# Illumina/strelka

Measured on AMD Instinct MI355X. Metric: candidate-alignment scoring cells/s (read bases x candidate alignments; Strelka2 has no pair-HMM, SURVEY.md section 0) + germline loci/s + 40x WGS-like germline wall-clock (e2e) + 110x/40x somatic wall-clock (e2e_somatic), higher is better.
Workload: dtype f64; 1 GPU; germline chr20-style synthetic (BASELINE.json configs[1]).  Headline: scoreCandidateAlignment as one function -- per GPU per step 65536 reads of 150 bp x 87.9 candidate alignments each (5-7 candidate indels around them), from the candidate alignments the device search left (PCal) to one double each: one kernel (F5: the walk of each alignment's path + the terms of its bases, penalties and clips).  ; read_len=150

## Files before the change

### strelka_amd/csrc/read_enumerate.hip

```cpp

#include "sk_common.h"

#include "align_entry.h"
#include "read_enumerate.h"

#include <algorithm>
#include <chrono>
#include <climits>
#include <cstdio>
#include <cstdlib>
#include <cstring>
#include <vector>

using namespace skcore;

int sk_score_alignments_launch_hostleg(const sk_align_batch* b, double* dev_out_lnp, void* hip_stream);

namespace
{

static_assert(sizeof(PFrame) % 4 == 0 && sizeof(PCal) % 4 == 0, "frames move through LDS as 32-bit words");


struct EnumArgs
// ... 457 lines not shown
    if (nc == 0) return;
    int32_t wb = a.win_begin[r], we = a.win_end[r];
    if (wb > we) wb = we = 0;
    a.win_begin[r] = wb;
    int32_t len = we - wb;
    a.win_len[r] = len;
    int16_t* idx = a.ins_idx + size_t(r) * INS_CAP;
    int32_t* off = a.ins_off + size_t(r) * INS_CAP;
    int n = 0;
    for (int t = a.ins_lo[r]; t <= a.ins_hi[r]; ++t) {
        const uint32_t il = a.job.tab[t].ins_len;
        if (il == 0) continue;
        if (n >= INS_CAP) {
            a.status[r] = ST_OVERFLOW;
            n = 0;
            break;
        }
        idx[n] = int16_t(t);
        off[n] = len;
        len += int32_t(il);
        ++n;
    }
    a.n_ins[r] = n;
    a.hap_len[r] = max(len, 1);
}

__device__ int matching_indel(const PJob& j, const PCal& c, const int32_t ref_head_pos, const unsigned del_len, const unsigned ins_len,
                              const int ends_first, const int ends_second, const int path_index)
{
    if (path_index < ends_first) return c.lead;
    if (path_index > ends_second) return c.trail;
    int found = -1;
    for (int k = 0; k < c.n_indels; ++k) {
        const PIndel& ci = j.tab[c.indels[k]];
        if (ci.pos == ref_head_pos && (ci.type == SK_INDEL_INDEL || ci.type == SK_INDEL_MISMATCH) && ci.del == del_len &&
            ci.ins_len == ins_len) {
            if (found >= 0) return -2;
            found = c.indels[k];
        } else if (ci.pos > ref_head_pos) {
            break;
        }
    }
    return found >= 0 ? found : -2;
}

struct NoOpSink
{
    __device__ __forceinline__ void operator()(uint8_t, uint32_t, int32_t, bool) const {}
};

template <bool WRITE, typename SINK = NoOpSink>
__device__ int flatten_cal(const FlatArgs& a, const int r, const PCal& c, const int32_t read_len, sk_score_op* ops, SINK&& sink = SINK())
{
    const int aps = c.n_seg;
    const int32_t win_begin = a.win_begin[r];
    const int n_ins = a.n_ins[r];
    const int16_t* ins_idx = a.ins_idx + size_t(r) * INS_CAP;
    const int32_t* ins_off = a.ins_off + size_t(r) * INS_CAP;
    unsigned read_offset = 0;
    int32_t ref_head_pos = c.pos;
    int ends_first = aps, ends_second = aps;
    {
        bool is_first_match = false;
        for (int i = 0; i < aps; ++i)
            if (seg_align_match(c.path[i].type)) {
                if (!is_first_match) ends_first = i;
                is_first_match = true;
                ends_second = i;
            }
    }
    int n = 0;
    auto emit = [&](const uint8_t kind, const uint32_t len, const int32_t src, const bool penalty) {
        if (kind == SK_OP_NOBASE && !penalty) return;
        sink(kind, len, src, penalty);
        if (WRITE) {
            sk_score_op op;
            op.length = uint16_t(len);
            op.kind = kind;
            op.flags = uint8_t(penalty ? SK_OPFLAG_NONCANDIDATE_PENALTY : 0);
            op.src = src;
            ops[n] = op;
        }
        ++n;
    };
    auto insert_src = [&](const int idx, const int32_t head, const uint32_t len) -> int32_t {
        const PIndel& k = a.job.tab[idx];
        if (head < 0 || uint32_t(head) + len > k.ins_len) return -1;
        for (int i = 0; i < n_ins; ++i)
            if (ins_idx[i] == idx) return ins_off[i] + head;
        return -1;
    };
    auto is_cand = [&](const int idx) -> bool { return job_cand(a.job, idx); };

    int path_index = 0;
    while (path_index < aps) {
        bool is_swap_start = false;
        {
            bool is_insert = false, is_delete = false;
            for (int i = path_index; i < aps; ++i) {
                if (c.path[i].type == SK_SEG_INSERT) is_insert = true;
                else if (c.path[i].type == SK_SEG_DELETE) is_delete = true;
                else break;
            }
            is_swap_start = is_insert && is_delete;
        }
        unsigned n_seg = 1;
        const PSeg ps = c.path[path_index];
        if (is_swap_start || ps.type == SK_SEG_SEQ_MISMATCH) {
            unsigned del_len, ins_len;
            if (ps.type == SK_SEG_SEQ_MISMATCH) {
                del_len = ins_len = ps.length;
            } else {
                int k = path_index;
                del_len = ins_len = 0;
                for (; k < aps && (c.path[k].type == SK_SEG_INSERT || c.path[k].type == SK_SEG_DELETE); ++k) {
                    if (c.path[k].type == SK_SEG_INSERT) ins_len += c.path[k].length;
                    else del_len += c.path[k].length;
                }
                n_seg = unsigned(k - path_index);
            }
            const int key = matching_indel(a.job, c, ref_head_pos, del_len, ins_len, ends_first, ends_second, path_index);
            if (key < 0) return -1;
            int32_t head = 0;
            if (path_index < ends_first) head = int32_t(a.job.tab[key].ins_len) - int32_t(ps.length);
            const bool pen = !is_cand(key);
            if (ins_len > 0) {
                if (ins_len > 0xffffu) return -1;
                const int32_t src = insert_src(key, head, ins_len);
                if (src < 0) return -1;
                emit(SK_OP_BASES, ins_len, src, pen);
            } else {
                emit(SK_OP_NOBASE, 0, 0, pen);
            }
        } else if (seg_align_match(ps.type)) {
            emit(SK_OP_BASES, ps.length, ref_head_pos - win_begin, false);
        } else if (ps.type == SK_SEG_INSERT) {
            const int key = matching_indel(a.job, c, ref_head_pos, 0, ps.length, ends_first, ends_second, path_index);
            if (key < 0) return -1;
            int32_t head = 0;
            if (path_index < ends_first) head = int32_t(a.job.tab[key].ins_len) - int32_t(ps.length);
            const int32_t src = insert_src(key, head, ps.length);
            if (src < 0) return -1;
            emit(SK_OP_BASES, ps.length, src, !is_cand(key));
        } else if (ps.type == SK_SEG_DELETE) {
            const int key = matching_indel(a.job, c, ref_head_pos, ps.length, 0, ends_first, ends_second, path_index);
            if (key < 0) return -1;
            emit(SK_OP_NOBASE, 0, 0, !is_cand(key));
        } else if (ps.type == SK_SEG_SKIP || ps.type == SK_SEG_HARD_CLIP) {
        } else if (ps.type == SK_SEG_SOFT_CLIP) {
            emit(SK_OP_SOFT_CLIP, ps.length, 0, false);
        } else {
            return -1;
        }
        for (unsigned i = 0; i < n_seg; ++i) {
            const PSeg s = c.path[path_index];
            if (seg_align_match(s.type)) {
                read_offset += s.length;
                ref_head_pos += int32_t(s.length);
            } else if (s.type == SK_SEG_DELETE || s.type == SK_SEG_SKIP) {
                ref_head_pos += int32_t(s.length);
            } else if (s.type == SK_SEG_INSERT || s.type == SK_SEG_SOFT_CLIP) {
                read_offset += s.length;
            }
            path_index++;
        }
    }
    if (int64_t(read_offset) != int64_t(read_len)) return -1;
    return n;
}

__global__ __launch_bounds__(64) void op_count_kernel(const FlatArgs a)
{
    const int c = blockIdx.x * blockDim.x + threadIdx.x;
    if (c >= a.n_cals) return;
    const int r = read_of_cal(a, c);
    const PCal& cal = a.pool[a.list[c]];
    const int n = flatten_cal<false>(a, r, cal, int32_t(a.read_off[r + 1] - a.read_off[r]), nullptr);
    if (n < 0) a.status[r] = ST_FAIL;
    a.n_ops[c] = n < 0 ? 0 : n;
}

__global__ __launch_bounds__(64) void pool_fill_kernel(const FlatArgs a)
{
    const int r = blockIdx.x;
    if (a.cal_off[r + 1] == a.cal_off[r]) return;
    uint8_t* hap = a.hap_code + a.hap_off[r];
    const int32_t P = int32_t(a.hap_off[r + 1] - a.hap_off[r]);
    const int32_t wb = a.win_begin[r];
    const int n_ins = a.n_ins[r];
    const int16_t* idx = a.ins_idx + size_t(r) * INS_CAP;
    const int32_t* off = a.ins_off + size_t(r) * INS_CAP;
    const int32_t win_len = a.win_len[r];
    for (int32_t i = threadIdx.x; i < P; i += 64) {
        uint8_t v = SK_BAM_ANY;
        if (i < win_len) {
            const int32_t p = wb + i;
            const bool outside = (p < a.ref_offset || p >= a.ref_offset + a.ref_len);
            if (outside && a.ref_outside) atomicAdd(a.ref_outside, 1);
            v = outside ? uint8_t(SK_BAM_ANY) : code_of(a.ref[p - a.ref_offset]);
        }
        for (int k = 0; k < n_ins; ++k) {
            const PIndel& d = a.job.tab[idx[k]];
            if (i >= off[k] && i < off[k] + int32_t(d.ins_len)) v = code_of(a.ins_pool[d.ins_off + uint32_t(i - off[k])]);
        }
        hap[i] = v;
    }
}

__global__ __launch_bounds__(64) void flatten_kernel(const FlatArgs a)
{
    constexpr int REC_DW = int(sizeof(PCal) / 4), REC_STRIDE = REC_DW | 1;
    static_assert(sizeof(PCal) % 4 == 0 && REC_DW <= 128, "a record is at most two dwords per lane");
    __shared__ uint32_t s_cal[64 * REC_STRIDE];
    const int lane = threadIdx.x;
    const int c0 = blockIdx.x * blockDim.x;
    const int c = c0 + lane;
    const int nc = min(64, a.n_cals - c0);
    const int src_k = (lane < nc) ? a.list[c0 + lane] : 0;
    for (int k = 0; k < nc; ++k) {
        const uint32_t* __restrict__ src = reinterpret_cast<const uint32_t*>(a.pool + __shfl(src_k, k));
        uint32_t* __restrict__ dst = reinterpret_cast<uint32_t*>(a.cals + (c0 + k));
        for (int j = lane; j < REC_DW; j += 64) {
            const uint32_t v = src[j];
            s_cal[k * REC_STRIDE + j] = v;
            dst[j] = v;
        }
    }
    __syncthreads();
    if (c >= a.n_cals) return;
    const int r = read_of_cal(a, c);
    const PCal& cal = *reinterpret_cast<const PCal*>(s_cal + lane * REC_STRIDE);
    if (a.status[r] != ST_OK) return;
    (void)flatten_cal<true>(a, r, cal, int32_t(a.read_off[r + 1] - a.read_off[r]), a.ops + a.op_off[c]);
    for (int i = 0; i < cal.n_indels; ++i) (void)job_cand(a.job, cal.indels[i]);
    if (cal.lead >= 0) (void)job_cand(a.job, cal.lead);
    if (cal.trail >= 0) (void)job_cand(a.job, cal.trail);
}

constexpr int F5_MAX_READ = 256;
constexpr int ONE_WAIT_MAX_READS = 16384;
constexpr int F5_MAX_POOL = 768;
#ifndef F5_SORT
#define F5_SORT 1
#endif
constexpr int F5_TAB = 32;

static_assert(F5_TAB <= 64, "the table copy is a lane an entry");

struct FusedScoreArgs
{
    FlatArgs f;
    const uint8_t* read_qual;
    const SkTables* tab;
    double* scores;
    unsigned* err;
    int32_t* n_unhandled;
    int32_t write_cals;
    unsigned long long* dbg;
    unsigned* queue;
};

constexpr int F5_SEGS = 16, F5_INDELS = 8;
constexpr int F5_SLOT = (F5_SEGS + 1) | 1;
__device__ __forceinline__ int f5_ent_word(const int k) { return k; }
constexpr int F5_ROW = 3;

struct F5Tab
{
    int32_t pos;
    uint32_t del, ins_len;
    uint32_t type_cand;
    int32_t ins_at;
};

template <int MAXR>
struct F5Lds
{
    uint8_t read[MAXR + 12];
    uint8_t hap[F5_MAX_POOL + 12];
    double row[(MAXR + 8) * F5_ROW];
    uint32_t slot[64 * F5_SLOT];
    F5Tab tab[F5_TAB];
};
static_assert(sizeof(F5Lds<152>) <= 10240, "sixteen waves of the short-read form to a CU");
static_assert(3 * 4 * sizeof(F5Lds<F5_MAX_READ>) <= 160 * 1024, "three four-wave blocks of the long-read form to a CU");
static_assert((152 + 12) % 4 == 0 && (F5_MAX_READ + 12) % 4 == 0 && (F5_MAX_POOL + 12) % 4 == 0, "the byte arrays' words stay aligned");
static_assert(INS_CAP <= 64, "a lane an insert");

struct F5Rec
{
    uint32_t w0, w1, w2;
    uint64_t types;
    uint64_t l0, l1, l2, l3;
    uint64_t ind;
    int ind_lo;
    __device__ __forceinline__ int32_t pos() const { return int32_t(w0); }
    __device__ __forceinline__ int lead() const { return int(int16_t(w1 & 0xffffu)); }
    __device__ __forceinline__ int trail() const { return int(int16_t(w1 >> 16)); }
    __device__ __forceinline__ int n_seg() const { return int((w2 >> 8) & 0xffu); }
    __device__ __forceinline__ int n_indels() const { return int((w2 >> 16) & 0xffu); }
    __device__ __forceinline__ int indel(const int k) const { return ind_lo + int(unsigned(ind >> (6 * k)) & 63u); }
};
static_assert(F5_TAB <= 64 && 6 * F5_INDELS <= 64, "an indel index in 6 bits, eight in one value");

template <typename LDS>
__device__ __forceinline__ int f5_walk_selects(LDS& S, const F5Rec c, const bool has, const int tab_lo, const int32_t win_begin, uint8_t* consulted,
                                               const int32_t L, const int32_t P, uint32_t* const myslot)
{
    constexpr uint64_t N1 = 0x1111111111111111ull;
    const uint64_t types = c.types, p_l0 = c.l0, p_l1 = c.l1, p_l2 = c.l2, p_l3 = c.l3;
    const int aps = has ? c.n_seg() : 0;
    auto eq4 = [=](const unsigned v) -> uint64_t {
        uint64_t x = types ^ (N1 * v);
        x |= x >> 1;
        x |= x >> 2;
        return ~x & N1;
    };
    auto seg_len = [=](const int i) -> unsigned {
        const uint64_t lo = (i & 4) ? p_l1 : p_l0, hi = (i & 4) ? p_l3 : p_l2;
        return unsigned(((i & 8) ? hi : lo) >> (16 * (i & 3))) & 0xffffu;
    };
    const uint64_t in_path = (aps >= 16) ? N1 : (((1ull << (4 * aps)) - 1ull) & N1);
    const uint64_t M4 = (eq4(SK_SEG_MATCH) | eq4(SK_SEG_SEQ_MATCH) | eq4(SK_SEG_SEQ_MISMATCH)) & in_path;
    const uint64_t I4 = eq4(SK_SEG_INSERT) & in_path, D4 = eq4(SK_SEG_DELETE) & in_path;
    const int ends_first = M4 ? (__builtin_ctzll(M4) >> 2) : aps, ends_second = M4 ? ((63 - __builtin_clzll(M4)) >> 2) : aps;
    const int ni = c.n_indels();
    int ni_wave = 0;
#pragma unroll
    for (int k = 1; k <= F5_INDELS; ++k) ni_wave = __any(ni >= k) ? k : ni_wave;
    int32_t k_pos[F5_INDELS];
    uint32_t k_pack[F5_INDELS];
    bool bad = false;
#pragma unroll
    for (int k = 0; k < F5_INDELS; ++k) {
        k_pos[k] = INT_MIN;
        k_pack[k] = 0xffffffffu;
        if (k < ni_wave) {
            const F5Tab& ci = S.tab[((k < ni) ? c.indel(k) : tab_lo) - tab_lo];
            const unsigned ty = ci.type_cand & 0xffu;
            const bool kind = (ty == SK_INDEL_INDEL || ty == SK_INDEL_MISMATCH);
            if (k < ni) {
                k_pos[k] = ci.pos;
                if (kind) {
                    k_pack[k] = (ci.del << 16) | ci.ins_len;
                    bad = bad || ci.del >= 0xffffu || ci.ins_len >= 0xffffu;
                }
            }
        }
    }
    int pi = 0, n_ent = 0;
    int32_t pos = 0, ref_head_pos = c.pos();
    unsigned npen = 0;
    for (;;) {
        const bool live = pi < aps && !bad;
        if (!__any(live)) break;
        const int sh = 4 * (pi & 15);
        const unsigned ty = unsigned(types >> sh) & 15u, ln = seg_len(pi & 15);
        const uint64_t not_run = ~((I4 | D4) >> sh) & N1;
        const int run4 = not_run ? __builtin_ctzll(not_run) : 64;
        const uint64_t run_set = (run4 >= 64) ? ~0ull : ((1ull << run4) - 1ull);
        const bool is_swap = live && ((I4 >> sh) & run_set) != 0ull && ((D4 >> sh) & run_set) != 0ull;
        const bool is_match = (ty == SK_SEG_MATCH || ty == SK_SEG_SEQ_MATCH), is_clip = (ty == SK_SEG_SOFT_CLIP);
        const bool is_indel_seg = is_swap || ty == SK_SEG_SEQ_MISMATCH || ty == SK_SEG_INSERT || ty == SK_SEG_DELETE;
        unsigned del_len = (ty == SK_SEG_INSERT) ? 0u : ln, ins_len = (ty == SK_SEG_DELETE) ? 0u : ln;
        int n_seg = 1;
        unsigned read_step = (is_match || ty == SK_SEG_SEQ_MISMATCH || ty == SK_SEG_INSERT || is_clip) ? ln : 0u;
        unsigned ref_step = (is_match || ty == SK_SEG_SEQ_MISMATCH || ty == SK_SEG_DELETE || ty == SK_SEG_SKIP) ? ln : 0u;
        if (is_swap) {
            n_seg = run4 >> 2;
            del_len = ins_len = 0;
            for (int k = 0; k < n_seg; ++k) {
                const unsigned l = seg_len((pi + k) & 15);
                if ((I4 >> (4 * ((pi + k) & 15))) & 1ull) ins_len += l;
                else del_len += l;
            }
            read_step = ins_len;
            ref_step = del_len;
        }
        const unsigned asked = (del_len << 16) | ins_len;
        const bool askable = del_len < 0xffffu && ins_len < 0xffffu;
        int k_found = 0, n_found = 0;
        bool open = true;
#pragma unroll
        for (int k = 0; k < F5_INDELS; ++k) {
            if (k < ni_wave) {
                const bool m = open && k_pos[k] == ref_head_pos && k_pack[k] == asked;
                k_found = m ? k : k_found;
                n_found += m ? 1 : 0;
                open = open && (m || k_pos[k] <= ref_head_pos);
            }
        }
        int key = (n_found == 1) ? c.indel(k_found) : -2;
        key = (pi < ends_first) ? c.lead() : (pi > ends_second) ? c.trail() : key;
        const bool key_ok = key >= 0;
        const F5Tab te = S.tab[(key_ok ? key : tab_lo) - tab_lo];
        const bool indel_ok = live && is_indel_seg && key_ok;
        if (indel_ok && consulted) consulted[key] = 1;
        const bool pen = is_indel_seg && (te.type_cand >> 8) == 0u;
        const int32_t head = (pi < ends_first) ? int32_t(te.ins_len) - int32_t(ln) : 0;
        const bool ins_bases = is_indel_seg && ins_len > 0u;
        const bool ins_ok = ins_len <= 0xffffu && head >= 0 && uint32_t(head) + ins_len <= te.ins_len && te.ins_at >= 0;
        const bool bases = ins_bases || is_match;
        const int32_t src = ins_bases ? te.ins_at + head : ref_head_pos - win_begin;
        const unsigned len = ins_bases ? ins_len : ln;
        const bool known = is_indel_seg || is_match || is_clip || ty == SK_SEG_SKIP || ty == SK_SEG_HARD_CLIP;
        bool fail = !known || (is_indel_seg && (!key_ok || !askable)) || (ins_bases && !ins_ok);
        const bool entry = (bases || (is_clip && !is_indel_seg)) && len > 0u;
        if (entry) {
            fail = fail || pos + int32_t(len) > L || (bases && (src < 0 || int64_t(src) + int64_t(len) > int64_t(P)));
            const int hidx = bases ? int(src) - pos : 0;
            fail = fail || n_ent > F5_SEGS || npen > 4u || hidx < -256 || hidx > 3839;
            if (live && !fail) myslot[f5_ent_word(n_ent)] = unsigned(pos) | (npen << 9) | (bases ? 0u : 1u << 15) | (unsigned(hidx + 256) << 16);
        }
        if (live) {
            bad = fail;
            n_ent += entry ? 1 : 0;
            npen = entry ? (pen ? 1u : 0u) : npen + (pen ? 1u : 0u);
            pos += int32_t(read_step);
            ref_head_pos += int32_t(ref_step);
            pi += n_seg;
        }
    }
    if (!has) return 0;
    if (bad || pos != L || n_ent > F5_SEGS || npen > 4u) return -1;
    myslot[f5_ent_word(n_ent)] = unsigned(L) | (npen << 9) | (256u << 16);
    return n_ent + 1;
}

template <typename LDS>
__device__ __forceinline__ double f5_sum(LDS& S, const uint32_t* const myslot, const int n_ent, const double ln_noncand, const double ln_quarter)
{
    double lnp = 0.0;
    const unsigned char* rows = reinterpret_cast<const unsigned char*>(S.row);
    int e = 0, p = 0, stop = 0, hidx = 0;
    uint32_t cur = myslot[f5_ent_word(0)], nxt = myslot[f5_ent_word(1)];
    auto next_op = [&]() -> bool {
        const bool adv = (p >= stop);
        const int start = int(cur & 0x1ffu), next_start = int(nxt & 0x1ffu);
        const unsigned np = adv ? ((cur >> 9) & 63u) : 0u;
        const bool clip = adv && (cur & (1u << 15)) != 0u;
        if (__builtin_amdgcn_ballot_w64(np != 0u || clip) != 0ull) {
            const double l1 = __dadd_rn(lnp, ln_noncand);
            lnp = (np >= 1u) ? l1 : lnp;
            const double l2 = __dadd_rn(lnp, ln_noncand);
            lnp = (np >= 2u) ? l2 : lnp;
            const double l3 = __dadd_rn(lnp, ln_noncand);
            lnp = (np >= 3u) ? l3 : lnp;
            const double l4 = __dadd_rn(lnp, ln_noncand);
            lnp = (np >= 4u) ? l4 : lnp;
            const double lc = __dadd_rn(lnp, __dmul_rn(double(unsigned(next_start - start)), ln_quarter));
            lnp = clip ? lc : lnp;
        }
        if (adv && e + 1 >= n_ent) return true;
        p = adv ? (clip ? next_start : start) : p;
        stop = adv ? next_start : stop;
        hidx = adv ? int(cur >> 16) - 256 : hidx;
        e = adv ? e + 1 : e;
        cur = adv ? nxt : cur;
        nxt = myslot[f5_ent_word(e + 1)];
        return false;
    };
    if (next_op()) return lnp;
    for (;;) {
        {
            const int m = stop - p;
            const int mm = (m > 8) ? 8 : m;
            const int ph = p + hidx;
            const uint32_t* const rw = reinterpret_cast<const uint32_t*>(S.read + (p & ~3));
            const uint32_t* const hw = reinterpret_cast<const uint32_t*>(S.hap + (ph & ~3));
            const uint32_t r0 = rw[0], r1 = rw[1], r2 = rw[2], h0 = hw[0], h1 = hw[1], h2 = hw[2];
            const uint32_t R[2] = {__builtin_amdgcn_alignbyte(r1, r0, unsigned(p)), __builtin_amdgcn_alignbyte(r2, r1, unsigned(p))};
            const uint32_t H[2] = {__builtin_amdgcn_alignbyte(h1, h0, unsigned(ph)), __builtin_amdgcn_alignbyte(h2, h1, unsigned(ph))};
            const uint64_t past = (mm >= 8) ? 0ull : (0x1818181818181818ull << (8 * mm));
            constexpr uint32_t B0F = 0x0f0f0f0fu, B10 = 0x10101010u;
            uint32_t sel[2];
#pragma unroll
            for (int h = 0; h < 2; ++h) {
                const uint32_t x = (R[h] ^ H[h]) + B0F;
                uint32_t pm = uint32_t(past >> (32 * h));
                __asm__("" : "+v"(pm));
                sel[h] = (B10 & ~pm & x) | (~B10 & pm);
                __asm__("" : "+v"(sel[h]));
            }
            const unsigned base = __umul24(unsigned(8 * F5_ROW), unsigned(p));
            double v[8];
#pragma unroll
            for (int u = 0; u < 8; ++u) {
                const unsigned at = base + unsigned(8 * F5_ROW * u) + ((sel[u >> 2] >> (8 * (u & 3))) & 0xffu);
                v[u] = *reinterpret_cast<const double*>(rows + at);
            }
#pragma unroll
            for (int u = 0; u < 8; ++u) lnp = __dadd_rn(lnp, v[u]);
            p += mm;
        }
        if (next_op()) break;
    }
    return lnp;
}

__device__ __forceinline__ void f5_wave_sync()
{
    __builtin_amdgcn_fence(__ATOMIC_RELEASE, "workgroup");
    __builtin_amdgcn_wave_barrier();
    __builtin_amdgcn_fence(__ATOMIC_ACQUIRE, "workgroup");
}

template <int MAXR, bool TIMING>
__device__ __forceinline__ void f5_read(const FusedScoreArgs& fa, const int r, F5Lds<MAXR>& S)
{
    auto now = [&]() -> unsigned long long { return TIMING ? (unsigned long long)clock64() : 0ull; };
    const FlatArgs& a = fa.f;
    const int lane = threadIdx.x & 63;
    const int c0 = a.cal_off[r], c1 = a.cal_off[r + 1];
    const int ncr = c1 - c0;
    if (ncr == 0 || a.status[r] != ST_OK) return;
    unsigned long long stamp[8];
    stamp[0] = now();
    const unsigned long long wall0 = TIMING ? (unsigned long long)wall_clock64() : 0ull;
    for (int i = 1; i < 8; ++i) stamp[i] = 0;
    const int64_t ro = a.read_off[r];
    const int32_t L = int32_t(a.read_off[r + 1] - ro);
    const int32_t P = a.hap_len[r];
    if (L > MAXR || P > F5_MAX_POOL) {
        if (lane == 0) atomicAdd(fa.n_unhandled, 1);
        return;
    }
    const int32_t win_begin = a.win_begin[r];
    const int n_ins = a.n_ins[r];
    int my_ins_idx = -1;
    int32_t my_ins_off = 0;
    {
        const int16_t* idx = a.ins_idx + size_t(r) * INS_CAP;
        const int32_t* off = a.ins_off + size_t(r) * INS_CAP;
        int32_t my_ins_len = 0;
        uint32_t my_ins_src = 0;
        if (lane < n_ins) {
            const int t_idx = idx[lane];
            my_ins_idx = t_idx;
            my_ins_off = off[lane];
            my_ins_len = int32_t(a.job.tab[t_idx].ins_len);
            my_ins_src = a.job.tab[t_idx].ins_off;
        }
        const int32_t win_len = a.win_len[r];
        for (int32_t i = lane; i < P + 8; i += 64) {
            uint8_t v = SK_BAM_ANY;
            if (i < win_len) {
                const int32_t p = win_begin + i;
                const bool outside = (p < a.ref_offset || p >= a.ref_offset + a.ref_len);
                if (outside && a.ref_outside) atomicAdd(a.ref_outside, 1);
                v = outside ? uint8_t(SK_BAM_ANY) : code_of(a.ref[p - a.ref_offset]);
            }
            S.hap[i] = v;
        }
        f5_wave_sync();
        for (int k = 0; k < n_ins; ++k) {
            const int32_t o = __builtin_amdgcn_readlane(my_ins_off, k), n = __builtin_amdgcn_readlane(my_ins_len, k);
            const uint32_t src = uint32_t(__builtin_amdgcn_readlane(int(my_ins_src), k));
            for (int32_t i = lane; i < n; i += 64)
                if (o + i < P) S.hap[o + i] = code_of(a.ins_pool[src + uint32_t(i)]);
        }
        const SkTables* __restrict__ T = fa.tab;
        for (int32_t i = lane; i < L + 12; i += 64) {
            unsigned q = 0;
            uint8_t code = SK_BAM_ANY;
            if (i < L) {
                code = a.read_code[ro + i];
                q = fa.read_qual[ro + i];
                if (q > 70u) {
                    atomicOr(fa.err, unsigned(SK_DEVERR_QSCORE));
                    q = 70u;
                }
            }
            S.read[i] = code & 15u;
            if (i < L + 8) {
                const unsigned c = code & 15u;
                const bool adds = i < L && c != 15u;
                const double agree = adds ? T->q2lncompe[q] : 0.0;
                S.row[F5_ROW * i] = agree;
                S.row[F5_ROW * i + 1] = 0.0;
                S.row[F5_ROW * i + 2] = !adds ? 0.0 : (c == 0u) ? agree : T->q2mis[q];
            }
        }
    }
    const double ln_quarter = fa.tab->ln_quarter, ln_noncand = fa.tab->ln_noncand;

    uint8_t* const order = S.hap + ((P + 8 + 3) & ~3);
    const bool sorted_order = (F5_SORT != 0) && ncr > 64 && ncr <= 256 && ((P + 8 + 3) & ~3) + ncr <= int(sizeof(S.hap));
    if (sorted_order) {
        int seg_of[4];
#pragma unroll
        for (int k = 0; k < 4; ++k) {
            const int j = lane + 64 * k;
            seg_of[k] = (j < ncr) ? int(a.n_seg8[c0 + j]) : -1;
            seg_of[k] = min(seg_of[k], F5_SEGS + 1);
        }
        unsigned present = 0;
#pragma unroll
        for (int k = 0; k < 4; ++k) present |= (seg_of[k] >= 0) ? (1u << seg_of[k]) : 0u;
#pragma unroll
        for (int d = 32; d >= 1; d >>= 1) present |= unsigned(__shfl_xor(int(present), d));
        present = unsigned(__builtin_amdgcn_readfirstlane(int(present)));
        int at = 0;
        while (present != 0u) {
            const int v = 31 - __builtin_clz(present);
            present &= ~(1u << v);
#pragma unroll
            for (int k = 0; k < 4; ++k) {
                const uint64_t m = __ballot(seg_of[k] == v);
                if (seg_of[k] == v) order[at + __popcll(m & ((1ull << lane) - 1ull))] = uint8_t(lane + 64 * k);
                at += __popcll(m);
            }
        }
    }

    for (int j0 = 0; j0 < ncr; j0 += 64) {
        const int nc = min(64, ncr - j0);
        f5_wave_sync();
        const unsigned long long ta = now();
        if (j0 == 0) stamp[1] = ta;
        const bool has = lane < nc;
        uint32_t* const myslot = S.slot + lane * F5_SLOT;
        bool fits = true;
        const int my_j = has ? (sorted_order ? int(order[j0 + lane]) : j0 + lane) : 0;
        F5Rec rec;
        rec.w0 = rec.w1 = rec.w2 = 0;
        rec.types = 0;
        rec.l0 = rec.l1 = rec.l2 = rec.l3 = 0;
        rec.ind = 0;
        rec.ind_lo = 0;
        uint64_t ind_raw0 = 0, ind_raw1 = 0;
        if (has) {
            const PCal* src = a.pool + a.list[c0 + my_j];
            const uint4* s4 = reinterpret_cast<const uint4*>(src);
            const uint4 q0 = s4[0], q1 = s4[1], q2 = s4[2], q3 = s4[3], q4 = s4[4];
            const uint32_t* si = reinterpret_cast<const uint32_t*>(src->indels);
            const uint32_t i0 = si[0], i1 = si[1], i2 = si[2], i3 = si[3];
            ind_raw0 = uint64_t(i0) | (uint64_t(i1) << 32);
            ind_raw1 = uint64_t(i2) | (uint64_t(i3) << 32);
            rec.w0 = q0.x;
            rec.w1 = q0.y;
            rec.w2 = q0.z;
            const unsigned nseg = (q0.z >> 8) & 0xffu, nind = (q0.z >> 16) & 0xffu;
            fits = (nseg <= unsigned(F5_SEGS) && nind <= unsigned(F5_INDELS));
            uint64_t types = 0;
            bool odd_type = false;
            auto pack4 = [&](const uint32_t a0, const uint32_t a1, const uint32_t a2, const uint32_t a3, const int first) -> uint64_t {
                types |= (uint64_t(a0 & 15u) | (uint64_t(a1 & 15u) << 4) | (uint64_t(a2 & 15u) << 8) | (uint64_t(a3 & 15u) << 12)) << (4 * first);
                odd_type = odd_type || (unsigned(first) < nseg && (a0 & 0xffffu) > 15u) || (unsigned(first + 1) < nseg && (a1 & 0xffffu) > 15u) ||
                           (unsigned(first + 2) < nseg && (a2 & 0xffffu) > 15u) || (unsigned(first + 3) < nseg && (a3 & 0xffffu) > 15u);
                return uint64_t(a0 >> 16) | (uint64_t(a1 >> 16) << 16) | (uint64_t(a2 >> 16) << 32) | (uint64_t(a3 >> 16) << 48);
            };
            rec.l0 = pack4(q0.w, q1.x, q1.y, q1.z, 0);
            rec.l1 = pack4(q1.w, q2.x, q2.y, q2.z, 4);
            rec.l2 = pack4(q2.w, q3.x, q3.y, q3.z, 8);
            rec.l3 = pack4(q3.w, q4.x, q4.y, q4.z, 12);
            rec.types = types;
            fits = fits && !odd_type;
        }
        auto raw_indel = [&](const int k) -> int { return int(int16_t(((k & 4) ? ind_raw1 : ind_raw0) >> (16 * (k & 3)))); };
        int tab_lo = 0;
        {
            int lo = INT_MAX, hi = INT_MIN;
            if (has && fits) {
                auto add = [&](const int i) {
                    lo = min(lo, i);
                    hi = max(hi, i);
                };
                const int ni = rec.n_indels();
                for (int i = 0; i < ni; ++i) add(raw_indel(i));
                if (rec.lead() >= 0) add(rec.lead());
                if (rec.trail() >= 0) add(rec.trail());
            }
#pragma unroll
            for (int d = 32; d > 0; d >>= 1) {
                lo = min(lo, __shfl_xor(lo, d));
                hi = max(hi, __shfl_xor(hi, d));
            }
            const int n_tab = (lo <= hi) ? hi - lo + 1 : 0;
            if (__any(has && !fits) || (n_tab > 0 && lo < 0) || n_tab > F5_TAB) {
                if (lane == 0) atomicAdd(fa.n_unhandled, 1);
                return;
            }
            tab_lo = n_tab ? lo : 0;
            uint64_t ind = 0;
#pragma unroll
            for (int k = 0; k < F5_INDELS; ++k) ind |= uint64_t(unsigned(raw_indel(k) - tab_lo) & 63u) << (6 * k);
            rec.ind = ind;
            rec.ind_lo = tab_lo;
            if (lane < n_tab) {
                const PIndel& g = a.job.tab[tab_lo + lane];
                F5Tab e;
                e.pos = g.pos;
                e.del = g.del;
                e.ins_len = g.ins_len;
                e.type_cand = unsigned(g.type) | (unsigned(g.cand) << 8);
                e.ins_at = -1;
                S.tab[lane] = e;
            }
            f5_wave_sync();
            if (my_ins_idx >= tab_lo && my_ins_idx < tab_lo + n_tab) S.tab[my_ins_idx - tab_lo].ins_at = my_ins_off;
        }
        f5_wave_sync();
        const unsigned long long tc = now();
        stamp[2] += tc - ta;
        int n_ent = 0;
        bool bad = false;
        {
            const unsigned long long tA0 = now();
            n_ent = f5_walk_selects(S, rec, has, tab_lo, win_begin, a.job.consulted, L, P, myslot);
            const unsigned long long tA1 = now();
            stamp[7] += tA1 - tA0;
            bad = n_ent < 0;
            if (has) {
                if (a.job.consulted) {
                    const int ni = rec.n_indels();
                    for (int i = 0; i < ni; ++i) a.job.consulted[rec.indel(i)] = 1;
                    if (rec.lead() >= 0) a.job.consulted[rec.lead()] = 1;
                    if (rec.trail() >= 0) a.job.consulted[rec.trail()] = 1;
                }
                if (bad) a.status[r] = ST_FAIL;
            }
            (void)tA1;
        }
        __builtin_amdgcn_wave_barrier();
        const unsigned long long td = now();
        stamp[4] += td - tc;
        if (has && !bad) {
            const double lnp = f5_sum(S, myslot, n_ent, ln_noncand, ln_quarter);
            fa.scores[c0 + my_j] = lnp;
        }
        stamp[5] += now() - td;
    }
    if (fa.dbg && lane == 0) {
        stamp[6] = now();
        stamp[3] = TIMING ? (unsigned long long)wall_clock64() - wall0 : 0ull;
        for (int i = 0; i < 8; ++i) fa.dbg[size_t(r) * 8 + i] = stamp[i];
    }
}

template <int MAXR, bool TIMING, int WAVES>
__global__ __launch_bounds__(64 * WAVES) __attribute__((amdgpu_waves_per_eu(4, 4))) void flatten_score_kernel(const FusedScoreArgs fa, const int n_reads)
{
    __shared__ __attribute__((aligned(16))) F5Lds<MAXR> S[WAVES];
    const int wave = threadIdx.x >> 6, lane = threadIdx.x & 63;
    for (;;) {
        int r = 0;
        if (lane == 0) r = int(atomicAdd(&fa.queue[0], 1u));
        r = __builtin_amdgcn_readfirstlane(r);
        if (r >= n_reads) break;
        f5_read<MAXR, TIMING>(fa, r, S[wave]);
        f5_wave_sync();
    }
    if (lane == 0) {
        __threadfence();
        if (atomicAdd(&fa.queue[1], 1u) == gridDim.x * unsigned(WAVES) - 1u) {
            fa.queue[0] = 0u;
            fa.queue[1] = 0u;
        }
    }
}

template <int MAXR, bool TIMING>
static void launch_flatten_score_t(const int n_reads, hipStream_t st, const FusedScoreArgs& fs)
{
    static const int waves = [] { const char* e = std::getenv("SK_F5_WAVES"); return e ? std::atoi(e) : 0; }();
    constexpr int DEFAULT_WAVES = (sizeof(F5Lds<MAXR>) * 16 <= 160 * 1024) ? 8 : 4;
    const int w = waves > 0 ? waves : DEFAULT_WAVES;
    static const int grid_env = [] { const char* e = std::getenv("SK_F5_GRID"); return e ? std::atoi(e) : 0; }();
    constexpr int WAVES_PER_CU = int((160 * 1024) / sizeof(F5Lds<MAXR>)) >= 16 ? 16 : int((160 * 1024) / sizeof(F5Lds<MAXR>));
    auto grid = [&](const int wpb) {
        const int resident = grid_env > 0 ? grid_env : 256 * std::max(1, WAVES_PER_CU / wpb);
        return dim3(unsigned(std::max(1, std::min(resident, (n_reads + wpb - 1) / wpb))));
    };
    if (w == 16 && MAXR <= 152) SK_LAUNCH((flatten_score_kernel<152, TIMING, 16>), grid(16), dim3(1024), 0, st, fs, n_reads);
    else if (w >= 8) SK_LAUNCH((flatten_score_kernel<MAXR, TIMING, 8>), grid(8), dim3(512), 0, st, fs, n_reads);
    else if (w == 4) SK_LAUNCH((flatten_score_kernel<MAXR, TIMING, 4>), grid(4), dim3(256), 0, st, fs, n_reads);
    else if (w == 2) SK_LAUNCH((flatten_score_kernel<MAXR, TIMING, 2>), grid(2), dim3(128), 0, st, fs, n_reads);
    else SK_LAUNCH((flatten_score_kernel<MAXR, TIMING, 1>), grid(1), dim3(64), 0, st, fs, n_reads);
}

static void launch_flatten_score(const int n_reads, hipStream_t st, const FusedScoreArgs& fs)
{
    const bool short_reads = fs.f.max_read_len <= 152, timing = fs.dbg != nullptr;
    if (short_reads && !timing) launch_flatten_score_t<152, false>(n_reads, st, fs);
    else if (short_reads) launch_flatten_score_t<152, true>(n_reads, st, fs);
    else if (!timing) launch_flatten_score_t<F5_MAX_READ, false>(n_reads, st, fs);
    else launch_flatten_score_t<F5_MAX_READ, true>(n_reads, st, fs);
}

__global__ __launch_bounds__(64) void gather_cals_kernel(const PCal* __restrict__ pool, const int32_t* __restrict__ list, const int32_t n_cals,
                                                         PCal* __restrict__ cals)
{
    constexpr int REC_DW = int(sizeof(PCal) / 4);
    const int lane = threadIdx.x;
    const int c0 = blockIdx.x * 64;
    const int nc = min(64, n_cals - c0);
    const int src_k = (lane < nc) ? list[c0 + lane] : 0;
    for (int k0 = 0; k0 < nc; k0 += 16) {
        uint32_t v0[16], v1[16];
#pragma unroll
        for (int u = 0; u < 16; ++u) {
            const int k = k0 + u;
            const uint32_t* __restrict__ src = reinterpret_cast<const uint32_t*>(pool + __shfl(src_k, (k < nc) ? k : 0));
            v0[u] = (k < nc) ? src[lane] : 0u;
            v1[u] = (k < nc && lane + 64 < REC_DW) ? src[lane + 64] : 0u;
        }
#pragma unroll
        for (int u = 0; u < 16; ++u) {
            const int k = k0 + u;
            if (k < nc) {
                uint32_t* __restrict__ dst = reinterpret_cast<uint32_t*>(cals + (c0 + k));
                dst[lane] = v0[u];
                if (lane + 64 < REC_DW) dst[lane + 64] = v1[u];
            }
        }
    }
}


__device__ inline bool f3_emit_entries(const FlatArgs& a, const int c, const int r, const uint8_t* hap, const int32_t L, const int32_t P,
                                       uint32_t* ent, int& n_ent)
{
    const int W = a.evmask_words;
    uint32_t* mask = a.evmask + int64_t(r) * W;
    const bool read_ok = (L >= 0 && L <= SK_ENT_MAX_READ_LEN && L <= a.max_read_len && P >= 0 && P <= SK_ENT_MAX_POOL);
    auto col_at = [&](const int idx) -> unsigned { return (idx >= 0 && idx < P) ? sk_ent_col_index(hap[idx]) : unsigned(SK_ENT_ZERO_COL); };
    const int64_t k0 = a.op_off[c], k1 = a.op_off[c + 1];
    const int nslots = int(k1 - k0) + 2;
    for (int i = 0; i < nslots; ++i) ent[i] = SK_ENT_END;
    bool complex_cal = !read_ok;
    int e = 0, pos = 0;
    unsigned npen = 0;
    auto emit = [&](const unsigned np, const bool clip, const int hidx) {
        if (np > 7u || hidx + SK_ENT_HIDX_BIAS < 0 || hidx + SK_ENT_HIDX_BIAS > 2047) complex_cal = true;
        if (complex_cal) return;
        ent[e++] = unsigned(pos) | (np << 10) | (clip ? 1u << 13 : 0u) | (col_at(hidx + pos) << 15) | (col_at(hidx + pos + 1) << 18) |
                   (unsigned(hidx + SK_ENT_HIDX_BIAS) << 21);
        if (pos > 0 && pos <= L) atomicOr(&mask[pos >> 5], 1u << (pos & 31));
    };
    for (int64_t kk = k0; kk < k1 && !complex_cal; ++kk) {
        const sk_score_op op = a.ops[kk];
        const int len = int(op.length);
        const unsigned pen = op.flags & SK_OPFLAG_NONCANDIDATE_PENALTY;
        if ((op.kind == SK_OP_BASES || op.kind == SK_OP_SOFT_CLIP) && len > 0) {
            if (pos >= int(SK_ENT_END)) {
                complex_cal = true;
                break;
            }
            const bool bases = (op.kind == SK_OP_BASES);
            if (bases && (op.src < 0 || int64_t(op.src) + len > P)) complex_cal = true;
            emit(npen, !bases, bases ? int(op.src) - pos : P - pos);
            pos += len;
            npen = pen;
        } else {
            npen += pen;
        }
    }
    if (!complex_cal) {
        if (pos != L || pos >= int(SK_ENT_END)) complex_cal = true;
        else emit(npen, false, P - pos);
    }
    if (complex_cal) {
        for (int i = 0; i < nslots; ++i) ent[i] = SK_ENT_END;
        ent[0] = SK_ENT_COMPLEX;
        atomicOr(&a.addmask[int64_t(r) * W + (W - 1)], 1u << 31);
        n_ent = 0;
        return true;
    }
    uint32_t* am = a.addmask + int64_t(r) * W;
    for (int i = 0; i < e; ++i)
        if (ent[i] & SK_ENT_ADD_BITS) {
            const unsigned p = ent[i] & SK_ENT_POS_MASK;
            atomicOr(&am[p >> 5], 1u << (p & 31));
        }
    n_ent = e;
    return false;
}

__device__ inline void f3_columns_serial(const FlatArgs& a, const int c, const int r, const uint8_t* hap, const int32_t L, const int32_t P,
                                         const uint32_t* ent, const int e)
{
    const int W = a.evmask_words;
    auto col_at = [&](const int idx) -> unsigned { return (idx >= 0 && idx < P) ? sk_ent_col_index(hap[idx]) : unsigned(SK_ENT_ZERO_COL); };
    const int64_t k0 = a.op_off[c], k1 = a.op_off[c + 1];
    const int ncr = a.cal_off[r + 1] - a.cal_off[r], j = c - a.cal_off[r];
    uint32_t* cm = reinterpret_cast<uint32_t*>(a.colmat) + a.colmat_off[r] + j;
    const uint8_t* read = a.read_code + a.read_off[r];
    constexpr uint32_t NONE_WORD = 0x11111111u * SK_SEL_NONE;
    uint32_t word = NONE_WORD;
    int wk = 0;
    int pos = 0;
    const int nch = (L + 7) >> 3;
    int ei = 0;
    bool needs_entries = false;
    auto flag_at = [&](const int i) -> unsigned {
        while (ei < e && int(ent[ei] & SK_ENT_POS_MASK) < i) ++ei;
        if (ei < e && int(ent[ei] & SK_ENT_POS_MASK) == i && (ent[ei] & SK_ENT_ADD_BITS)) {
            const bool simple = ((ent[ei] >> 10) & 7u) == 1u && !(ent[ei] & (1u << 13)) && i < 8 * nch;
            if (simple) return 4u;
            needs_entries = true;
        }
        return 0u;
    };
    auto put = [&](const int i, const unsigned sel) {
        const int k8 = i >> 3;
        if (k8 != wk) {
            cm[int64_t(wk) * ncr] = word;
            for (int q = wk + 1; q < k8; ++q) cm[int64_t(q) * ncr] = NONE_WORD;
            word = NONE_WORD;
            wk = k8;
        }
        const unsigned shift = 8u * (unsigned(i) & 3u) + ((i & 4) ? 4u : 0u);
        word = (word & ~(0xfu << shift)) | (sel << shift);
    };
    for (int64_t kk = k0; kk < k1; ++kk) {
        const sk_score_op op = a.ops[kk];
        const int len = int(op.length);
        if (!((op.kind == SK_OP_BASES || op.kind == SK_OP_SOFT_CLIP) && len > 0)) continue;
        if (op.kind == SK_OP_BASES) {
            for (int t = 0; t < len && pos + t < L; ++t)
                put(pos + t, sk_col_selector(col_at(int(op.src) + t), read[pos + t]) | flag_at(pos + t));
        } else if (flag_at(pos)) {
        }
        pos += len;
    }
    {
        const unsigned f = flag_at(L);
        if (f) put(L, SK_SEL_NONE | f);
    }
    for (; ei < e; ++ei)
        if ((ent[ei] & SK_ENT_ADD_BITS) && int(ent[ei] & SK_ENT_POS_MASK) > L) needs_entries = true;
    if (needs_entries) atomicOr(&a.addmask[int64_t(r) * W + (W - 1)], 1u << 30);
    if (wk < nch) cm[int64_t(wk) * ncr] = word;
    for (int q = wk + 1; q < nch; ++q) cm[int64_t(q) * ncr] = NONE_WORD;
}

__global__ __launch_bounds__(64) void entries_kernel(const FlatArgs a)
{
    const int c = blockIdx.x * blockDim.x + threadIdx.x;
    if (c >= a.n_cals) return;
    const int r = read_of_cal(a, c);
    const int32_t L = int32_t(a.read_off[r + 1] - a.read_off[r]);
    const int32_t P = int32_t(a.hap_off[r + 1] - a.hap_off[r]);
    const uint8_t* hap = a.hap_code + a.hap_off[r];
    uint32_t* ent = a.entries + a.op_off[c] + 2 * int64_t(c);
    int e = 0;
    if (f3_emit_entries(a, c, r, hap, L, P, ent, e)) return;
    f3_columns_serial(a, c, r, hap, L, P, ent, e);
}

constexpr int F3W_MAX_D = 64;
constexpr int F3W_MAX_NCH = 32;
constexpr int F3W_MAX_POOL = 1024;

struct F3wLds
{
    uint8_t hap[F3W_MAX_POOL];
    uint8_t read[8 * F3W_MAX_NCH];
    uint8_t slot_of[2048];
    uint32_t delta_bits[64];
    int32_t n_slots;
    int16_t delta_of[F3W_MAX_D];
    uint32_t M[F3W_MAX_D][F3W_MAX_NCH];
    uint32_t tile[F3W_MAX_NCH][64];
};

__device__ __forceinline__ uint32_t f3w_below(const int x)
{
    const uint32_t lo = (x >= 4) ? 0x0f0f0f0fu : (uint32_t((1ull << (8 * x)) - 1ull) & 0x0f0f0f0fu);
    const uint32_t hi = (x <= 4) ? 0u : (x >= 8 ? 0xf0f0f0f0u : (uint32_t((1ull << (8 * (x - 4))) - 1ull) & 0xf0f0f0f0u));
    return lo | hi;
}

__global__ __launch_bounds__(64) void entries_wave_kernel(const FlatArgs a)
{
    __shared__ F3wLds S;
    const int r = blockIdx.x;
    const int lane = threadIdx.x;
    const int c0 = a.cal_off[r], c1 = a.cal_off[r + 1];
    const int ncr = c1 - c0;
    if (ncr == 0) return;
    const int32_t L = int32_t(a.read_off[r + 1] - a.read_off[r]);
    const int32_t P = int32_t(a.hap_off[r + 1] - a.hap_off[r]);
    const uint8_t* ghap = a.hap_code + a.hap_off[r];
    const uint8_t* gread = a.read_code + a.read_off[r];
    const int nch = (L + 7) >> 3;
    const bool fits = (L >= 0 && nch <= F3W_MAX_NCH && P >= 0 && P <= F3W_MAX_POOL);
    if (fits) {
        for (int i = lane; i < P; i += 64) S.hap[i] = ghap[i];
        for (int i = lane; i < 8 * nch; i += 64) S.read[i] = (i < L) ? gread[i] : uint8_t(15);
    }
    S.delta_bits[lane] = 0;
    if (lane == 0) S.n_slots = 0;
    __syncthreads();
    const uint8_t* hap = fits ? S.hap : ghap;

    for (int c = c0 + lane; c < c1; c += 64) {
        uint32_t* ent = a.entries + a.op_off[c] + 2 * int64_t(c);
        int e = 0;
        const bool complex_cal = f3_emit_entries(a, c, r, hap, L, P, ent, e);
        if (complex_cal) continue;
        if (!fits) {
            f3_columns_serial(a, c, r, hap, L, P, ent, e);
            continue;
        }
        int pos = 0;
        for (int64_t kk = a.op_off[c]; kk < a.op_off[c + 1]; ++kk) {
            const sk_score_op op = a.ops[kk];
            const int len = int(op.length);
            if (!((op.kind == SK_OP_BASES || op.kind == SK_OP_SOFT_CLIP) && len > 0)) continue;
            if (op.kind == SK_OP_BASES) {
                const int d = int(op.src) - pos + SK_ENT_HIDX_BIAS;
                atomicOr(&S.delta_bits[d >> 5], 1u << (d & 31));
            }
            pos += len;
        }
    }
    if (!fits) return;
    __syncthreads();
    {
        const uint32_t w = S.delta_bits[lane];
        int n = __popc(w), before = n;
#pragma unroll
        for (int d = 1; d < 64; d <<= 1) {
// ... 1269 lines not shown
```

Baseline: 757.1 billion cells/s.

## Add swap-free fast path for alignment walk and batch consulted-flag writes per wave

```diff
diff --git a/strelka_amd/csrc/read_enumerate.hip b/strelka_amd/csrc/read_enumerate.hip
--- a/strelka_amd/csrc/read_enumerate.hip
+++ b/strelka_amd/csrc/read_enumerate.hip
@@ -783,10 +783,17 @@
     __device__ __forceinline__ int indel(const int k) const { return ind_lo + int(unsigned(ind >> (6 * k)) & 63u); }
 };
 static_assert(F5_TAB <= 64 && 6 * F5_INDELS <= 64, "an indel index in 6 bits, eight in one value");
+static_assert(F5_TAB <= 32, "the entries a round names as one 32-bit set");
+
+constexpr unsigned F5_T_MATCH = (1u << SK_SEG_MATCH) | (1u << SK_SEG_SEQ_MATCH), F5_T_CLIP = 1u << SK_SEG_SOFT_CLIP;
+constexpr unsigned F5_T_INDEL = (1u << SK_SEG_SEQ_MISMATCH) | (1u << SK_SEG_INSERT) | (1u << SK_SEG_DELETE);
+constexpr unsigned F5_T_KNOWN = F5_T_MATCH | F5_T_INDEL | F5_T_CLIP | (1u << SK_SEG_SKIP) | (1u << SK_SEG_HARD_CLIP);
+constexpr unsigned F5_T_READ = F5_T_MATCH | (1u << SK_SEG_SEQ_MISMATCH) | (1u << SK_SEG_INSERT) | F5_T_CLIP;
+constexpr unsigned F5_T_REF = F5_T_MATCH | (1u << SK_SEG_SEQ_MISMATCH) | (1u << SK_SEG_DELETE) | (1u << SK_SEG_SKIP);
 
 template <typename LDS>
-__device__ __forceinline__ int f5_walk_selects(LDS& S, const F5Rec c, const bool has, const int tab_lo, const int32_t win_begin, uint8_t* consulted,
-                                               const int32_t L, const int32_t P, uint32_t* const myslot)
+__device__ __forceinline__ int f5_walk_selects(LDS& S, const F5Rec c, const bool has, const int tab_lo, const int32_t win_begin, const int32_t L,
+                                               const int32_t P, uint32_t* const myslot)
 {
     constexpr uint64_t N1 = 0x1111111111111111ull;
     const uint64_t types = c.types, p_l0 = c.l0, p_l1 = c.l1, p_l2 = c.l2, p_l3 = c.l3;
@@ -832,7 +839,69 @@
     int pi = 0, n_ent = 0;
     int32_t pos = 0, ref_head_pos = c.pos();
     unsigned npen = 0;
-    for (;;) {
+    const bool no_swap = !__any((((I4 << 4) & D4) | ((D4 << 4) & I4)) != 0ull);
+#pragma unroll 1
+    for (int w = 0; no_swap && w < F5_SEGS / 4; ++w) {
+        if (!__any(4 * w < aps && !bad)) break;
+        const unsigned tw = unsigned(types >> (16 * w)) & 0xffffu;
+        const uint64_t lw = (w == 0) ? p_l0 : (w == 1) ? p_l1 : (w == 2) ? p_l2 : p_l3;
+#pragma unroll
+        for (int j = 0; j < 4; ++j) {
+            const int t = 4 * w + j;
+            const bool live = t < aps && !bad;
+            if (j > 0 && !__any(live)) break;
+            const unsigned ty = (tw >> (4 * j)) & 15u, ln = unsigned(lw >> (16 * j)) & 0xffffu;
+            auto in = [=](const unsigned set) -> bool { return ((set >> ty) & 1u) != 0u; };
+            const bool is_match = in(F5_T_MATCH), is_clip = in(F5_T_CLIP), is_indel_seg = in(F5_T_INDEL);
+            const unsigned del_len = (ty == SK_SEG_INSERT) ? 0u : ln, ins_len = (ty == SK_SEG_DELETE) ? 0u : ln;
+            const bool before = t < ends_first, after = t > ends_second;
+            int key = before ? c.lead() : c.trail();
+            if (__any(live && is_indel_seg && !before && !after)) {
+                const uint64_t asked = (uint64_t(uint32_t(ref_head_pos)) << 32) | uint64_t((del_len << 16) | ins_len);
+                int sh_found = 0, n_found = 0;
+                bool open = true;
+                auto look = [&](const int k) {
+                    const bool m = open && ((uint64_t(uint32_t(k_pos[k])) << 32) | uint64_t(k_pack[k])) == asked;
+                    sh_found = m ? 6 * k : sh_found;
+                    n_found += m ? 1 : 0;
+                    open = open && k_pos[k] <= ref_head_pos;
+                };
+#pragma unroll
+                for (int k = 0; k < F5_INDELS / 2; ++k) look(k);
+                if (ni_wave > F5_INDELS / 2) {
+#pragma unroll
+                    for (int k = F5_INDELS / 2; k < F5_INDELS; ++k) look(k);
+                }
+                const int between = (n_found == 1) ? c.ind_lo + int(unsigned(c.ind >> sh_found) & 63u) : -2;
+                key = (before || after) ? key : between;
+            }
+            const bool key_ok = key >= 0;
+            const F5Tab te = S.tab[(key_ok ? key : tab_lo) - tab_lo];
+            const bool pen = is_indel_seg && (te.type_cand >> 8) == 0u;
+            const int32_t head = before ? int32_t(te.ins_len) - int32_t(ln) : 0;
+            const bool ins_bases = is_indel_seg && ins_len > 0u;
+            const bool ins_ok = head >= 0 && uint32_t(head) + ins_len <= te.ins_len && te.ins_at >= 0;
+            const bool bases = ins_bases || is_match;
+            const int32_t src = ins_bases ? te.ins_at + head : ref_head_pos - win_begin;
+            const unsigned len = ins_bases ? ins_len : ln;
+            bool fail = !in(F5_T_KNOWN) || (is_indel_seg && (!key_ok || ln == 0xffffu)) || (ins_bases && !ins_ok);
+            const bool entry = (bases || is_clip) && len > 0u;
+            if (entry) {
+                fail = fail || pos + int32_t(len) > L || (bases && (src < 0 || int64_t(src) + int64_t(len) > int64_t(P)));
+                const int hidx = bases ? int(src) - pos : 0;
+                fail = fail || n_ent > F5_SEGS || npen > 4u || hidx < -256 || hidx > 3839;
+                if (live && !fail) myslot[f5_ent_word(n_ent)] = unsigned(pos) | (npen << 9) | (bases ? 0u : 1u << 15) | (unsigned(hidx + 256) << 16);
+            }
+            if (live) {
+                bad = fail;
+                n_ent += entry ? 1 : 0;
+                npen = entry ? (pen ? 1u : 0u) : npen + (pen ? 1u : 0u);
+                pos += int32_t(in(F5_T_READ) ? ln : 0u);
+                ref_head_pos += int32_t(in(F5_T_REF) ? ln : 0u);
+            }
+        }
+    }
+    while (!no_swap) {
         const bool live = pi < aps && !bad;
         if (!__any(live)) break;
         const int sh = 4 * (pi & 15);
@@ -875,8 +944,6 @@
         key = (pi < ends_first) ? c.lead() : (pi > ends_second) ? c.trail() : key;
         const bool key_ok = key >= 0;
         const F5Tab te = S.tab[(key_ok ? key : tab_lo) - tab_lo];
-        const bool indel_ok = live && is_indel_seg && key_ok;
-        if (indel_ok && consulted) consulted[key] = 1;
         const bool pen = is_indel_seg && (te.type_cand >> 8) == 0u;
         const int32_t head = (pi < ends_first) ? int32_t(te.ins_len) - int32_t(ln) : 0;
         const bool ins_bases = is_indel_seg && ins_len > 0u;
@@ -1104,7 +1171,8 @@
         bool fits = true;
         const int my_j = has ? (sorted_order ? int(order[j0 + lane]) : j0 + lane) : 0;
         F5Rec rec;
-        rec.w0 = rec.w1 = rec.w2 = 0;
+        rec.w0 = rec.w2 = 0;
+        rec.w1 = 0xffffffffu;
         rec.types = 0;
         rec.l0 = rec.l1 = rec.l2 = rec.l3 = 0;
         rec.ind = 0;
@@ -1139,7 +1207,7 @@
             fits = fits && !odd_type;
         }
         auto raw_indel = [&](const int k) -> int { return int(int16_t(((k & 4) ? ind_raw1 : ind_raw0) >> (16 * (k & 3)))); };
-        int tab_lo = 0;
+        int tab_lo = 0, n_tab = 0;
         {
             int lo = INT_MAX, hi = INT_MIN;
             if (has && fits) {
@@ -1157,7 +1225,7 @@
                 lo = min(lo, __shfl_xor(lo, d));
                 hi = max(hi, __shfl_xor(hi, d));
             }
-            const int n_tab = (lo <= hi) ? hi - lo + 1 : 0;
+            n_tab = __builtin_amdgcn_readfirstlane((lo <= hi) ? hi - lo + 1 : 0);
             if (__any(has && !fits) || (n_tab > 0 && lo < 0) || n_tab > F5_TAB) {
                 if (lane == 0) atomicAdd(fa.n_unhandled, 1);
                 return;
@@ -1188,19 +1256,24 @@
         bool bad = false;
         {
             const unsigned long long tA0 = now();
-            n_ent = f5_walk_selects(S, rec, has, tab_lo, win_begin, a.job.consulted, L, P, myslot);
+            n_ent = f5_walk_selects(S, rec, has, tab_lo, win_begin, L, P, myslot);
             const unsigned long long tA1 = now();
             stamp[7] += tA1 - tA0;
             bad = n_ent < 0;
-            if (has) {
-                if (a.job.consulted) {
+            if (a.job.consulted) {
+                uint32_t named = 0;
+                if (has) {
                     const int ni = rec.n_indels();
-                    for (int i = 0; i < ni; ++i) a.job.consulted[rec.indel(i)] = 1;
-                    if (rec.lead() >= 0) a.job.consulted[rec.lead()] = 1;
-                    if (rec.trail() >= 0) a.job.consulted[rec.trail()] = 1;
+                    for (int i = 0; i < ni; ++i) named |= 1u << (unsigned(rec.ind >> (6 * i)) & 31u);
+                    if (rec.lead() >= 0) named |= 1u << unsigned(rec.lead() - tab_lo);
+                    if (rec.trail() >= 0) named |= 1u << unsigned(rec.trail() - tab_lo);
                 }
-                if (bad) a.status[r] = ST_FAIL;
-            }
+#pragma unroll
+                for (int d = 32; d > 0; d >>= 1) named |= uint32_t(__shfl_xor(int(named), d));
+                const uint32_t all = uint32_t(__builtin_amdgcn_readfirstlane(int(named)));
+                if (lane < n_tab && __builtin_amdgcn_ubfe(all, unsigned(lane), 1u)) a.job.consulted[tab_lo + lane] = 1;
+            }
+            if (has && bad) a.status[r] = ST_FAIL;
             (void)tA1;
         }
         __builtin_amdgcn_wave_barrier();
```

Measured after the change: 763.5 billion cells/s, median of 6. About the same (+0.8%).
